# vovach777/llcomp

Measured on AMD Instinct MI355X. Metric: encode+decode MPix/s on 4K RGB8, bit-exact, higher is better.
Workload: dtype int32

## Files before the change

### llcomp_amd/csrc/model_kernels.hip

```cpp
#include <algorithm>

#include "device_common.hpp"
#include "kernels.hpp"

namespace llcomp_mi {

namespace {

constexpr int kMW = 256;
constexpr int kMH = 32;

template <int C>
__device__ __forceinline__ void rct_forward(const uint8_t* p, int16_t (&o)[C]) {
    if constexpr (C >= 3) {
        const int g = p[1], cb = int(p[2]) - g, cr = int(p[0]) - g;
        o[0] = int16_t(cr);
        o[1] = int16_t(g + (cb + cr) / 4);
        o[2] = int16_t(cb);
        if constexpr (C == 4) o[3] = p[3];
    } else {
#pragma unroll
        for (int k = 0; k < C; ++k) o[k] = p[k];
    }
}
// ... 651 lines not shown
struct RowTile {
    unsigned long long base;
    uint32_t sw;
};
template <int C>
__device__ __forceinline__ void load_row_tiles(const Geometry& g, uint32_t first_tile, uint32_t ntiles, RowTile* tiles) {
    if (threadIdx.x < ntiles) {
        const uint32_t tile = first_tile + threadIdx.x;
        const uint32_t per_frame = g.ntx * g.nty;
        const uint32_t frame = tile / per_frame, rem = tile - frame * per_frame;
        const uint32_t y = rem / g.ntx, tx = rem - y * g.ntx;
        const uint32_t x0 = tx * g.tile_w;
        tiles[threadIdx.x].base = ((size_t(frame) * g.h + y) * g.w + x0) * C;
        tiles[threadIdx.x].sw = g.w - x0 < g.tile_w ? g.w - x0 : g.tile_w;
    }
}

typedef short s16x2 __attribute__((ext_vector_type(2)));
typedef unsigned short u16x2 __attribute__((ext_vector_type(2)));
__device__ __forceinline__ u16x2 pk_min_u16(u16x2 a, u16x2 b) {
    u16x2 d;
    asm("v_pk_min_u16 %0, %1, %2" : "=v"(d) : "v"(a), "v"(b));
    return d;
}

template <int C>
__global__ __launch_bounds__(256) void k_model_rows_fwd(const Geometry g, const uint8_t* __restrict__ px,
                                                        uint16_t* __restrict__ lanes) {
    constexpr int K = 64, RUN = (K + 2) * C, TPG = 64 / C + 2;
    constexpr int RUNW = (RUN + 3) / 4 + 1;
    constexpr int PADL = (C - 1 + 1) & ~1, OCOLS = (PADL + 64 + C - 1 + 1) & ~1;
    __shared__ uint32_t raw[TPG][RUNW + 1];
    __shared__ __attribute__((aligned(4))) uint16_t otile[K][OCOLS];
    __shared__ RowTile tiles[TPG];
    const uint32_t chunks = (g.tile_w + K - 1) / K;
    uint32_t group, chunk;
    if (!xcd_group_chunk((g.n_slices + (1u << g.lane_shift) - 1) >> g.lane_shift, chunks, group, chunk)) return;
    const uint32_t k0 = chunk * K;
    const uint32_t gw = 1u << g.lane_shift;
    const uint32_t first_id = group << g.lane_shift;
    const uint32_t end_id = first_id + gw < g.n_slices ? first_id + gw : g.n_slices;
    const uint32_t first_tile = first_id / C, ntiles = (end_id - 1) / C - first_tile + 1;
    load_row_tiles<C>(g, first_tile, ntiles, tiles);
    __syncthreads();
    const size_t total_bytes = size_t(g.frames) * g.h * g.w * C;
    const uint32_t lane = threadIdx.x & 63, wave = threadIdx.x >> 6;
    constexpr int TPW = (TPG + 3) / 4, DPT = (RUNW + 63) / 64;
    uint32_t got[TPW][DPT];
#pragma unroll
    for (int t = 0; t < TPW; ++t) {
        const uint32_t tt = wave + 4 * t;
#pragma unroll
        for (int e = 0; e < DPT; ++e) got[t][e] = 0;
        if (tt < ntiles) {
            const long long start = (long long)tiles[tt].base + (long long)(int(k0) - 2) * C;
            const unsigned long long a0u = (unsigned long long)(start & ~3ll);
            const long long a0 = (long long)((unsigned long long)uint32_t(__builtin_amdgcn_readfirstlane(uint32_t(a0u))) |
                                             ((unsigned long long)uint32_t(__builtin_amdgcn_readfirstlane(uint32_t(a0u >> 32))) << 32));
            if (a0 >= 0 && size_t(a0) + 4 * size_t(RUNW) <= total_bytes) {
#pragma unroll
                for (int e = 0; e < DPT; ++e) {
                    const uint32_t d = lane + 64 * e;
                    if (d < uint32_t(RUNW)) __builtin_memcpy(&got[t][e], px + a0 + 4 * d, 4);
                }
            } else {
#pragma unroll
                for (int e = 0; e < DPT; ++e) {
                    const long long al = a0 + 4ll * (lane + 64 * e);
                    if (al >= 0 && size_t(al) + 4 <= total_bytes) __builtin_memcpy(&got[t][e], px + al, 4);
                    else if (al >= 0 && size_t(al) < total_bytes) got[t][e] = load_bytes_le(px + al, uint32_t(total_bytes - size_t(al)));
                }
            }
        }
    }
#pragma unroll
    for (int t = 0; t < TPW; ++t) {
        const uint32_t tt = wave + 4 * t;
#pragma unroll
        for (int e = 0; e < DPT; ++e) {
            const uint32_t d = lane + 64 * e;
            if (tt < ntiles && d < uint32_t(RUNW)) raw[tt][d] = got[t][e];
        }
    }
    __syncthreads();
    const uint32_t q = threadIdx.x & 7;
    const bool small = (g.flags & kGeoSmallModel) != 0;
    for (uint32_t tt = threadIdx.x >> 3; tt < ntiles; tt += 32) {
        const uint32_t sw = tiles[tt].sw;
        const uint32_t kb = k0 + 8 * q;
        if (kb >= sw) continue;
        const uint32_t skew = uint32_t(((long long)tiles[tt].base + (long long)(int(k0) - 2) * C) & 3);
        const uint8_t* p = reinterpret_cast<const uint8_t*>(&raw[tt][0]) + skew + 8 * q * C;
        s16x2 V[C][5];
#pragma unroll
        for (int j = 0; j < 5; ++j) {
            const uint8_t* a = p + 2 * j * C;
            if constexpr (C >= 3) {
                const s16x2 R = {short(a[0]), short(a[C])}, G = {short(a[1]), short(a[C + 1])}, B = {short(a[2]), short(a[C + 2])};
                const s16x2 cr = R - G, cb = B - G, sum = cb + cr;
                V[0][j] = cr;
                V[1][j] = G + ((sum + ((sum >> 15) & short(3))) >> 2);
                V[2][j] = cb;
                if constexpr (C == 4) V[3][j] = s16x2{short(a[3]), short(a[C + 3])};
            } else {
#pragma unroll
                for (int ch = 0; ch < C; ++ch) V[ch][j] = s16x2{short(a[ch]), short(a[C + ch])};
            }
        }
        uint32_t first_mask = ~0u;
        if (kb == 0) {
            first_mask = 0;
#pragma unroll
            for (int ch = 0; ch < C; ++ch) V[ch][0] = s16x2{128, 128};
        }
        if (small) first_mask = 0;
        const uint32_t colp = uint32_t(int((first_tile + tt) * C) - int(first_id) + PADL);
#pragma unroll
        for (int m = 0; m < 4; ++m) {
#pragma unroll
            for (int ch = 0; ch < C; ++ch) {
                const s16x2 cur = V[ch][m + 1], Lp = V[ch][m];
                const s16x2 lp = {V[ch][m].y, V[ch][m + 1].x};
                s16x2 dq = Lp - lp;
                uint32_t dqb = __builtin_bit_cast(uint32_t, dq) & ((m == 0 || small) ? first_mask : ~0u);
                dq = __builtin_bit_cast(s16x2, dqb);
                const s16x2 neg = dq >> 15;
                const u16x2 aq = __builtin_bit_cast(u16x2, (dq ^ neg) - neg);
                const u16x2 one = {1, 1};
                const u16x2 cidx = pk_min_u16(aq, one) + pk_min_u16(aq >> 2, one);
                const s16x2 res = ((cur - lp) ^ neg) - neg;
                const u16x2 sym = (__builtin_bit_cast(u16x2, res) & (unsigned short)0xFFF) + (cidx << 12);
                otile[8 * q + 2 * m][colp + ch] = sym.x;
                otile[8 * q + 2 * m + 1][colp + ch] = sym.y;
            }
        }
    }
    __syncthreads();
    if (g.lane_shift == 6) {
        for (uint32_t i = threadIdx.x; i < uint32_t(K) * 32; i += 256) {
            const uint32_t kk = i >> 5, d = i & 31, k = k0 + kk;
            if (k < g.tile_w)
                *reinterpret_cast<uint32_t*>(lanes + lane_order_index(g, first_id + 2 * d, k)) =
                    *reinterpret_cast<const uint32_t*>(&otile[kk][PADL + 2 * d]);
        }
    } else {
        for (uint32_t i = threadIdx.x; i < uint32_t(K) * gw; i += 256) {
            const uint32_t kk = i / gw, col = i - kk * gw, k = k0 + kk;
            if (k < g.tile_w && first_id + col < end_id) lanes[lane_order_index(g, first_id + col, k)] = otile[kk][PADL + col];
        }
    }
}

template <int C>
__global__ __launch_bounds__(256) void k_model_rows_inv(const Geometry g, const int16_t* __restrict__ lanes,
                                                        uint8_t* __restrict__ px) {
    constexpr int K = 64, TPG = 64 / C + 2;
    __shared__ __attribute__((aligned(4))) int16_t tile[K][64 + C + 1 + ((C + 1) & 1)];
    __shared__ RowTile tiles[TPG];
    const uint32_t chunks = (g.tile_w + K - 1) / K;
    uint32_t group, chunk;
    if (!xcd_chunk_group((g.n_slices + (1u << g.lane_shift) - 1) >> g.lane_shift, chunks, group, chunk)) return;
    const uint32_t k0 = chunk * K;
    const uint32_t gw = 1u << g.lane_shift;
    const uint32_t first_id = group << g.lane_shift;
    const uint32_t end_id = first_id + gw < g.n_slices ? first_id + gw : g.n_slices;
    const uint32_t first_tile = (first_id + C - 1) / C;
    const uint32_t end_tile = (end_id + C - 1) / C;
    if (first_tile >= end_tile) return;
    const uint32_t ntiles = end_tile - first_tile;
    load_row_tiles<C>(g, first_tile, ntiles, tiles);
    {
        uint32_t w[K * 32 / 256];
#pragma unroll
        for (int it = 0; it < K * 32 / 256; ++it) {
            const uint32_t i = threadIdx.x + 256 * it, kk = i >> 5, d = i & 31, k = k0 + kk;
            w[it] = 0;
            if (k < g.tile_w && g.lane_shift == 6)
                w[it] = *reinterpret_cast<const uint32_t*>(lanes + lane_order_index(g, first_id + 2 * d, k));
        }
        static_assert(K * (C - 1) <= 256, "one extra lane sample per thread");
        const uint32_t xk = threadIdx.x / (C > 1 ? C - 1 : 1), xe = threadIdx.x - xk * (C - 1);
        int16_t x = 0;
        if constexpr (C > 1) {
            const uint32_t id = first_id + gw + xe;
            if (xk < uint32_t(K) && id < g.n_slices && k0 + xk < g.tile_w) x = lanes[lane_order_index(g, id, k0 + xk)];
        }
#pragma unroll
        for (int it = 0; it < K * 32 / 256; ++it) {
            const uint32_t i = threadIdx.x + 256 * it, kk = i >> 5, d = i & 31;
            *reinterpret_cast<uint32_t*>(&tile[kk][2 * d]) = w[it];
        }
        if (g.lane_shift != 6) {
            __syncthreads();
            for (uint32_t i = threadIdx.x; i < uint32_t(K) * gw; i += 256) {
                const uint32_t kk = i / gw, col = i - kk * gw, k = k0 + kk;
                tile[kk][col] = (first_id + col < g.n_slices && k < g.tile_w) ? lanes[lane_order_index(g, first_id + col, k)] : int16_t(0);
            }
        }
        if constexpr (C > 1) {
            if (xk < uint32_t(K)) tile[xk][gw + xe] = x;
        }
    }
    __syncthreads();
    const uint32_t col0 = first_tile * C - first_id;
    const uint32_t q4 = threadIdx.x & 15;
    for (uint32_t tt = threadIdx.x >> 4; tt < ntiles; tt += 16) {
        const uint32_t sw = tiles[tt].sw, kb = k0 + 4 * q4;
        if (kb >= sw) continue;
        uint8_t bytes[4 * C];
#pragma unroll
        for (int i = 0; i < 4; ++i) {
            const int16_t* s = &tile[4 * q4 + i][col0 + tt * C];
            if constexpr (C >= 3) {
                int r = s[0], gg = s[1], bb = s[2];
                gg -= (r + bb) / 4;
                r += gg;
                bb += gg;
                bytes[i * C + 0] = uint8_t(min(max(r, 0), 255));
                bytes[i * C + 1] = uint8_t(min(max(gg, 0), 255));
                bytes[i * C + 2] = uint8_t(min(max(bb, 0), 255));
                if constexpr (C == 4) bytes[i * C + 3] = uint8_t(s[3]);
            } else {
#pragma unroll
                for (int c = 0; c < C; ++c) bytes[i * C + c] = uint8_t(s[c]);
            }
        }
        uint8_t* o = px + tiles[tt].base + size_t(kb) * C;
        const uint32_t npx = sw - kb < 4 ? sw - kb : 4;
        if (npx == 4) {
            uint32_t w[C];
#pragma unroll
            for (int c = 0; c < C; ++c)
                w[c] = uint32_t(bytes[4 * c]) | (uint32_t(bytes[4 * c + 1]) << 8) | (uint32_t(bytes[4 * c + 2]) << 16) |
                       (uint32_t(bytes[4 * c + 3]) << 24);
            __builtin_memcpy(o, w, 4 * C);
        } else {
            for (uint32_t i = 0; i < npx * C; ++i) o[i] = bytes[i];
        }
    }
}

struct RowTileCrop {
    long long base;
    uint32_t klo, khi;
};
template <int C>
__device__ __forceinline__ void load_row_tiles_crop(const Geometry& g, uint32_t first_tile, uint32_t ntiles, const Crop& cr,
                                                    RowTileCrop* tiles) {
    if (threadIdx.x < ntiles) {
        const uint32_t tile = first_tile + threadIdx.x;
        const uint32_t per_frame = g.ntx * g.nty;
        const uint32_t frame = tile / per_frame, rem = tile - frame * per_frame;
        const uint32_t y = rem / g.ntx, tx = rem - y * g.ntx;
        const uint32_t x0 = tx * g.tile_w;
        const uint32_t sw = g.w - x0 < g.tile_w ? g.w - x0 : g.tile_w;
        const uint32_t klo = cr.x0 > x0 ? cr.x0 - x0 : 0u;
        uint32_t khi = cr.x0 + cr.rw > x0 ? min(sw, cr.x0 + cr.rw - x0) : 0u;
        if (y < cr.y0 || y >= cr.y0 + cr.rh || khi <= klo) khi = 0;
        tiles[threadIdx.x].base = ((long long)(size_t(frame) * cr.rh + (y - cr.y0)) * cr.rw + (long long)x0 - (long long)cr.x0) * C;
        tiles[threadIdx.x].klo = klo;
        tiles[threadIdx.x].khi = khi;
    }
}
template <int C>
__global__ __launch_bounds__(256) void k_model_rows_inv_crop(const Geometry g, const int16_t* __restrict__ lanes,
                                                             uint8_t* __restrict__ px, const Crop cr) {
    constexpr int K = 64, TPG = 64 / C + 2;
    __shared__ __attribute__((aligned(4))) int16_t tile[K][64 + C + 1 + ((C + 1) & 1)];
    __shared__ RowTileCrop tiles[TPG];
    const uint32_t chunks = (g.tile_w + K - 1) / K;
    uint32_t group, chunk;
    if (!xcd_chunk_group((g.n_slices + (1u << g.lane_shift) - 1) >> g.lane_shift, chunks, group, chunk)) return;
    const uint32_t k0 = chunk * K;
    const uint32_t gw = 1u << g.lane_shift;
    const uint32_t first_id = group << g.lane_shift;
    const uint32_t end_id = first_id + gw < g.n_slices ? first_id + gw : g.n_slices;
    const uint32_t first_tile = (first_id + C - 1) / C;
    const uint32_t end_tile = (end_id + C - 1) / C;
    if (first_tile >= end_tile) return;
    const uint32_t ntiles = end_tile - first_tile;
    load_row_tiles_crop<C>(g, first_tile, ntiles, cr, tiles);
    {
        uint32_t w[K * 32 / 256];
#pragma unroll
        for (int it = 0; it < K * 32 / 256; ++it) {
            const uint32_t i = threadIdx.x + 256 * it, kk = i >> 5, d = i & 31, k = k0 + kk;
            w[it] = 0;
            if (k < g.tile_w && g.lane_shift == 6)
                w[it] = *reinterpret_cast<const uint32_t*>(lanes + lane_order_index(g, first_id + 2 * d, k));
        }
#pragma unroll
        for (int it = 0; it < K * 32 / 256; ++it) {
            const uint32_t i = threadIdx.x + 256 * it, kk = i >> 5, d = i & 31;
            *reinterpret_cast<uint32_t*>(&tile[kk][2 * d]) = w[it];
        }
    }
    if (g.lane_shift != 6) {
        __syncthreads();
        for (uint32_t i = threadIdx.x; i < uint32_t(K) * gw; i += 256) {
            const uint32_t kk = i / gw, col = i - kk * gw, k = k0 + kk;
            tile[kk][col] = (first_id + col < g.n_slices && k < g.tile_w) ? lanes[lane_order_index(g, first_id + col, k)] : int16_t(0);
        }
    }
    if constexpr (C > 1) {
        for (uint32_t i = threadIdx.x; i < uint32_t(K) * (C - 1); i += 256) {
            const uint32_t kk = i / (C - 1), e = i - kk * (C - 1), k = k0 + kk;
            const uint32_t id = first_id + gw + e;
            tile[kk][gw + e] = (id < g.n_slices && k < g.tile_w) ? lanes[lane_order_index(g, id, k)] : int16_t(0);
        }
    }
    __syncthreads();
    const uint32_t col0 = first_tile * C - first_id;
    const uint32_t q4 = threadIdx.x & 15;
    for (uint32_t tt = threadIdx.x >> 4; tt < ntiles; tt += 16) {
        const uint32_t sw = tiles[tt].khi, klo = tiles[tt].klo, kb = k0 + 4 * q4;
        if (kb >= sw || kb + 4 <= klo) continue;
        uint8_t bytes[4 * C];
#pragma unroll
        for (int i = 0; i < 4; ++i) {
            const int16_t* s = &tile[4 * q4 + i][col0 + tt * C];
            if constexpr (C >= 3) {
                int r = s[0], gg = s[1], bb = s[2];
                gg -= (r + bb) / 4;
                r += gg;
                bb += gg;
                bytes[i * C + 0] = uint8_t(min(max(r, 0), 255));
                bytes[i * C + 1] = uint8_t(min(max(gg, 0), 255));
                bytes[i * C + 2] = uint8_t(min(max(bb, 0), 255));
                if constexpr (C == 4) bytes[i * C + 3] = uint8_t(s[3]);
            } else {
#pragma unroll
                for (int c = 0; c < C; ++c) bytes[i * C + c] = uint8_t(s[c]);
            }
        }
        const uint32_t npx = sw - kb < 4 ? sw - kb : 4;
        if (npx < 4 || kb < klo) {
            for (uint32_t i = kb < klo ? klo - kb : 0u; i < npx; ++i)
                for (uint32_t c = 0; c < uint32_t(C); ++c) px[tiles[tt].base + (long long)(kb + i) * C + c] = bytes[i * C + c];
            continue;
        }
        uint32_t w[C];
#pragma unroll
        for (int c = 0; c < C; ++c)
            w[c] = uint32_t(bytes[4 * c]) | (uint32_t(bytes[4 * c + 1]) << 8) | (uint32_t(bytes[4 * c + 2]) << 16) |
                   (uint32_t(bytes[4 * c + 3]) << 24);
        __builtin_memcpy(px + tiles[tt].base + size_t(kb) * C, w, 4 * C);
    }
}



__global__ __launch_bounds__(256) void k_regions_index(const Geometry full, const Geometry sub, const RegionsFrame* __restrict__ tab,
                                                       const uint32_t* __restrict__ slice_len, const uint64_t* __restrict__ group_off,
                                                       uint32_t* __restrict__ sub_len, uint64_t* __restrict__ sub_off) {
    const uint32_t j = blockIdx.x * 256 + threadIdx.x;
    if (j >= sub.n_slices) return;
    const uint32_t id = regions_full_id(full, sub, tab, j);
    unsigned long long o = group_off[id >> full.lane_shift];
    for (uint32_t i = id & ~((1u << full.lane_shift) - 1); i < id; ++i) o += slice_len[i];
    sub_len[j] = slice_len[id];
    sub_off[j] = o;
}

template <int C>
__global__ __launch_bounds__(256) void k_model_inv_crops(const Geometry g, const int16_t* __restrict__ rec, uint8_t* __restrict__ px,
                                                         const RegionsFrame* __restrict__ tab, uint32_t rw, uint32_t rh, size_t npix) {
    const uint32_t c = C ? uint32_t(C) : g.c;
    const size_t per_frame = size_t(rw) * rh;
    for (size_t i = size_t(blockIdx.x) * blockDim.x + threadIdx.x; i < npix; i += size_t(gridDim.x) * blockDim.x) {
        const uint32_t f = uint32_t(i / per_frame);
        const uint32_t rem = uint32_t(i - f * per_frame), yy = rem / rw, xx = rem - yy * rw;
        const uint32_t y = tab[f].cy0 + yy, x = tab[f].cx0 + xx;
        uint8_t* o = px + (size_t(tab[f].out) * per_frame + rem) * c;
        uint32_t k = 0;
        if (c >= 3) {
            int r = rec[sample_index(g, f, y, x, 0)], gg = rec[sample_index(g, f, y, x, 1)], b = rec[sample_index(g, f, y, x, 2)];
            gg -= (r + b) / 4;
            r += gg;
            b += gg;
            o[0] = uint8_t(min(max(r, 0), 255));
            o[1] = uint8_t(min(max(gg, 0), 255));
            o[2] = uint8_t(min(max(b, 0), 255));
            k = 3;
        }
        for (; k < c; ++k) o[k] = uint8_t(rec[sample_index(g, f, y, x, k)]);
    }
}

template <int C>
__device__ __forceinline__ void load_row_tiles_crops(const Geometry& g, uint32_t first_tile, uint32_t ntiles, const RegionsFrame* tab,
                                                     uint32_t rw, uint32_t rh, RowTileCrop* tiles) {
    if (threadIdx.x < ntiles) {
        const uint32_t tile = first_tile + threadIdx.x;
        const uint32_t per_frame = g.ntx * g.nty;
        const uint32_t frame = tile / per_frame, rem = tile - frame * per_frame;
        const uint32_t y = rem / g.ntx, tx = rem - y * g.ntx;
        const uint32_t x0 = tx * g.tile_w;
        const uint32_t sw = g.w - x0 < g.tile_w ? g.w - x0 : g.tile_w;
        const uint32_t cx0 = tab[frame].cx0, cy0 = tab[frame].cy0;
        const uint32_t klo = cx0 > x0 ? cx0 - x0 : 0u;
        uint32_t khi = cx0 + rw > x0 ? min(sw, cx0 + rw - x0) : 0u;
        if (y < cy0 || y >= cy0 + rh || khi <= klo) khi = 0;
        tiles[threadIdx.x].base = ((long long)(size_t(tab[frame].out) * rh + (y - cy0)) * rw + (long long)x0 - (long long)cx0) * C;
        tiles[threadIdx.x].klo = klo;
        tiles[threadIdx.x].khi = khi;
    }
}
template <int C>
__global__ __launch_bounds__(256) void k_model_rows_inv_crops(const Geometry g, const int16_t* __restrict__ lanes,
                                                              uint8_t* __restrict__ px, const RegionsFrame* __restrict__ tab,
                                                              uint32_t rw, uint32_t rh) {
    constexpr int K = 64, TPG = 64 / C + 2;
    __shared__ __attribute__((aligned(4))) int16_t tile[K][64 + C + 1 + ((C + 1) & 1)];
    __shared__ RowTileCrop tiles[TPG];
    const uint32_t chunks = (g.tile_w + K - 1) / K;
    uint32_t group, chunk;
    if (!xcd_chunk_group((g.n_slices + (1u << g.lane_shift) - 1) >> g.lane_shift, chunks, group, chunk)) return;
    const uint32_t k0 = chunk * K;
    const uint32_t gw = 1u << g.lane_shift;
    const uint32_t first_id = group << g.lane_shift;
    const uint32_t end_id = first_id + gw < g.n_slices ? first_id + gw : g.n_slices;
    const uint32_t first_tile = (first_id + C - 1) / C;
    const uint32_t end_tile = (end_id + C - 1) / C;
    if (first_tile >= end_tile) return;
    const uint32_t ntiles = end_tile - first_tile;
    load_row_tiles_crops<C>(g, first_tile, ntiles, tab, rw, rh, tiles);
    {
        uint32_t w[K * 32 / 256];
#pragma unroll
        for (int it = 0; it < K * 32 / 256; ++it) {
            const uint32_t i = threadIdx.x + 256 * it, kk = i >> 5, d = i & 31, k = k0 + kk;
            w[it] = 0;
            if (k < g.tile_w && g.lane_shift == 6)
                w[it] = *reinterpret_cast<const uint32_t*>(lanes + lane_order_index(g, first_id + 2 * d, k));
        }
#pragma unroll
        for (int it = 0; it < K * 32 / 256; ++it) {
            const uint32_t i = threadIdx.x + 256 * it, kk = i >> 5, d = i & 31;
            *reinterpret_cast<uint32_t*>(&tile[kk][2 * d]) = w[it];
        }
    }
    if (g.lane_shift != 6) {
        __syncthreads();
        for (uint32_t i = threadIdx.x; i < uint32_t(K) * gw; i += 256) {
            const uint32_t kk = i / gw, col = i - kk * gw, k = k0 + kk;
            tile[kk][col] = (first_id + col < g.n_slices && k < g.tile_w) ? lanes[lane_order_index(g, first_id + col, k)] : int16_t(0);
        }
    }
    if constexpr (C > 1) {
        for (uint32_t i = threadIdx.x; i < uint32_t(K) * (C - 1); i += 256) {
            const uint32_t kk = i / (C - 1), e = i - kk * (C - 1), k = k0 + kk;
            const uint32_t id = first_id + gw + e;
            tile[kk][gw + e] = (id < g.n_slices && k < g.tile_w) ? lanes[lane_order_index(g, id, k)] : int16_t(0);
        }
    }
    __syncthreads();
    const uint32_t col0 = first_tile * C - first_id;
    const uint32_t q4 = threadIdx.x & 15;
    for (uint32_t tt = threadIdx.x >> 4; tt < ntiles; tt += 16) {
        const uint32_t sw = tiles[tt].khi, klo = tiles[tt].klo, kb = k0 + 4 * q4;
        if (kb >= sw || kb + 4 <= klo) continue;
        uint8_t bytes[4 * C];
#pragma unroll
        for (int i = 0; i < 4; ++i) {
            const int16_t* s = &tile[4 * q4 + i][col0 + tt * C];
            if constexpr (C >= 3) {
                int r = s[0], gg = s[1], bb = s[2];
                gg -= (r + bb) / 4;
                r += gg;
                bb += gg;
                bytes[i * C + 0] = uint8_t(min(max(r, 0), 255));
                bytes[i * C + 1] = uint8_t(min(max(gg, 0), 255));
                bytes[i * C + 2] = uint8_t(min(max(bb, 0), 255));
                if constexpr (C == 4) bytes[i * C + 3] = uint8_t(s[3]);
            } else {
#pragma unroll
                for (int c = 0; c < C; ++c) bytes[i * C + c] = uint8_t(s[c]);
            }
        }
        const uint32_t npx = sw - kb < 4 ? sw - kb : 4;
        if (npx < 4 || kb < klo) {
            for (uint32_t i = kb < klo ? klo - kb : 0u; i < npx; ++i)
                for (uint32_t c = 0; c < uint32_t(C); ++c) px[tiles[tt].base + (long long)(kb + i) * C + c] = bytes[i * C + c];
            continue;
        }
        uint32_t w[C];
#pragma unroll
        for (int c = 0; c < C; ++c)
            w[c] = uint32_t(bytes[4 * c]) | (uint32_t(bytes[4 * c + 1]) << 8) | (uint32_t(bytes[4 * c + 2]) << 16) |
                   (uint32_t(bytes[4 * c + 3]) << 24);
        __builtin_memcpy(px + tiles[tt].base + size_t(kb) * C, w, 4 * C);
    }
}


}

#define LLMI_DISPATCH_C(c, CALL) \
    switch (c) {                 \
        case 1: { constexpr int C = 1; CALL; } break; \
        case 2: { constexpr int C = 2; CALL; } break; \
        case 3: { constexpr int C = 3; CALL; } break; \
        case 4: { constexpr int C = 4; CALL; } break; \
        default: return hipErrorInvalidValue; \
    }

hipError_t launch_model_fwd(const Geometry& g, const uint8_t* d_px, uint32_t* d_sym, hipStream_t stream) {
    if (g.c > 4) {
        const size_t npix = size_t(g.frames) * g.h * g.w;
        k_model_fwd_any<<<dim3(uint32_t((npix + 255) / 256)), dim3(256), 0, stream>>>(g, d_px, d_sym, npix);
        return hipGetLastError();
    }
    const uint32_t nbx = (g.w + kMW - 1) / kMW;
    const uint32_t spt = (g.tile_h + kMH - 1) / kMH;
    const uint64_t blocks = uint64_t(nbx) * spt * g.nty * g.frames;
    if (blocks == 0 || blocks > 0x7FFFFFFFull) return hipErrorInvalidValue;
    LLMI_DISPATCH_C(g.c, (k_model_fwd<C><<<dim3(uint32_t(blocks)), dim3(kMW), 0, stream>>>(g, d_px, d_sym)));
    return hipGetLastError();
}

uint32_t lane_groups(const Geometry& g) { return (g.n_slices + (1u << g.lane_shift) - 1) >> g.lane_shift; }
uint32_t slice_capacity_samples(const Geometry& g) { return g.slice_samples; }

hipError_t launch_to_lane_order_u32(const Geometry& g, const uint32_t* d_img, uint32_t* d_lanes, hipStream_t stream) {
    const uint32_t max_n = slice_capacity_samples(g);
    const uint64_t blocks = uint64_t(lane_groups(g)) * ((max_n + 63) / 64);
    if (blocks == 0 || blocks > 0x7FFFFFFFull) return hipErrorInvalidValue;
    k_to_lane_order<uint32_t><<<dim3(uint32_t(blocks)), dim3(256), 0, stream>>>(g, max_n, d_img, d_lanes);
    return hipGetLastError();
}

hipError_t launch_from_lane_order_i16(const Geometry& g, const int16_t* d_lanes, int16_t* d_img, hipStream_t stream) {
    const uint32_t max_n = slice_capacity_samples(g);
    const uint64_t blocks = uint64_t(lane_groups(g)) * ((max_n + 63) / 64);
    if (blocks == 0 || blocks > 0x7FFFFFFFull) return hipErrorInvalidValue;
    k_from_lane_order<int16_t><<<dim3(uint32_t(blocks)), dim3(256), 0, stream>>>(g, max_n, d_lanes, d_img);
    return hipGetLastError();
}

bool model_is_fused(const Geometry& g) { return g.planar && rows_mode(g) && g.c <= 4; }
bool rows_encoder_reads_pixels(const Geometry& g) {
    return model_is_fused(g) && (uint64_t(63 / g.c + 2) * g.tile_w * g.c + 4 < (1ull << 31));
}

hipError_t launch_model_rows_fwd(const Geometry& g, const uint8_t* d_px, uint16_t* d_lanes, hipStream_t stream) {
    const uint64_t blocks = xcd_grid(lane_groups(g), (g.tile_w + 63) / 64);
    if (blocks == 0 || blocks > 0x7FFFFFFFull) return hipErrorInvalidValue;
    LLMI_DISPATCH_C(g.c, (k_model_rows_fwd<C><<<dim3(uint32_t(blocks)), dim3(256), 0, stream>>>(g, d_px, d_lanes)));
    return hipGetLastError();
}

hipError_t launch_model_rows_inv(const Geometry& g, const int16_t* d_lanes, uint8_t* d_px, hipStream_t stream) {
    const uint64_t blocks = xcd_chunk_grid(lane_groups(g), (g.tile_w + 63) / 64);
    if (blocks == 0 || blocks > 0x7FFFFFFFull) return hipErrorInvalidValue;
    LLMI_DISPATCH_C(g.c, (k_model_rows_inv<C><<<dim3(uint32_t(blocks)), dim3(256), 0, stream>>>(g, d_lanes, d_px)));
    return hipGetLastError();
}

hipError_t launch_model_inv(const Geometry& g, const int16_t* d_rec, uint8_t* d_px, hipStream_t stream) {
    const size_t npix = size_t(g.frames) * g.h * g.w;
    if (g.c > 4) {
        k_model_inv_any<<<dim3(uint32_t((npix + 255) / 256)), dim3(256), 0, stream>>>(g, d_rec, d_px, npix);
        return hipGetLastError();
    }
    const uint32_t blocks = uint32_t(std::min<size_t>((npix + 255) / 256, 256 * 16));
    LLMI_DISPATCH_C(g.c, (k_model_inv<C><<<dim3(blocks), dim3(256), 0, stream>>>(g, d_rec, d_px, npix)));
    return hipGetLastError();
}

hipError_t launch_group_sums(const Geometry& g, const uint32_t* d_slice_len, uint64_t* d_group_off, hipStream_t stream) {
    k_group_sums<<<dim3((g.n_slices + kSumThreads - 1) / kSumThreads), dim3(kSumThreads), 0, stream>>>(d_slice_len, g.n_slices, g.lane_shift, d_group_off);
    return hipGetLastError();
}

hipError_t launch_frame_bytes(const Geometry& g, const uint32_t* d_slice_len, uint64_t* d_frame_bytes, hipStream_t stream) {
    k_frame_bytes<<<dim3(g.frames), dim3(256), 0, stream>>>(d_slice_len, g.slices_per_frame, d_frame_bytes);
    return hipGetLastError();
}

hipError_t launch_scan_groups(const Geometry& g, uint64_t* d_group_off, uint64_t* d_total, hipStream_t stream) {
    k_scan_groups<<<dim3(1), dim3(kScanThreads), 0, stream>>>(d_group_off, lane_groups(g), d_total);
    return hipGetLastError();
}

hipError_t launch_copy_segments(const uint8_t* d_src, uint8_t* d_dst, const uint64_t* d_src_off, const uint64_t* d_dst_off,
                                const uint64_t* d_len, uint32_t n_seg, uint64_t max_len, hipStream_t stream) {
    if (n_seg == 0) return hipSuccess;
    if (n_seg > 65535) return hipErrorInvalidValue;
    const uint64_t pieces = (max_len / 4 + kSegPieceDwords - 1) / kSegPieceDwords;
    const uint32_t gx = uint32_t(std::min<uint64_t>(std::max<uint64_t>(pieces, 1), 1024));
    k_copy_segments<<<dim3(gx, n_seg), dim3(256), 0, stream>>>(d_src, d_dst, d_src_off, d_dst_off, d_len);
    return hipGetLastError();
}

hipError_t launch_range_sums(const uint32_t* d_vals, const uint64_t* d_start, const uint64_t* d_count, uint64_t* d_out, uint32_t n,
                             uint32_t cap, hipStream_t stream) {
    if (!n) return hipSuccess;
    k_range_sums<<<dim3(n), dim3(256), 0, stream>>>(d_vals, d_start, d_count, d_out, cap);
    return hipGetLastError();
}

hipError_t launch_pack_payload(const Geometry& g, const uint8_t* d_units, const uint32_t* d_slice_len,
                               const uint64_t* d_offsets, uint8_t* d_payload, uint64_t payload_cap,
                               uint32_t* d_status, hipStream_t stream) {
    k_pack_payload<<<dim3(lane_groups(g)), dim3(256), 0, stream>>>(g, reinterpret_cast<const uint4*>(d_units), d_slice_len,
                                                                   d_offsets, d_payload, payload_cap, d_status);
    return hipGetLastError();
}

hipError_t launch_region_index(const Geometry& full, const Geometry& sub, const RegionBox& box, const uint32_t* d_slice_len,
                               const uint64_t* d_group_off, uint32_t* d_sub_len, uint64_t* d_sub_off, hipStream_t stream) {
    if (sub.n_slices == 0) return hipErrorInvalidValue;
    k_region_index<<<dim3((sub.n_slices + 255) / 256), dim3(256), 0, stream>>>(full, sub, box, d_slice_len, d_group_off, d_sub_len, d_sub_off);
    return hipGetLastError();
}

hipError_t launch_stage_region_streams(const Geometry& sub, const uint8_t* d_payload, uint64_t payload_bytes, const uint32_t* d_sub_len,
                                       const uint64_t* d_sub_off, uint8_t* d_units, uint32_t* d_status, hipStream_t stream) {
    k_stage_region_streams<<<dim3(lane_groups(sub)), dim3(256), 0, stream>>>(sub, d_payload, payload_bytes, d_sub_len, d_sub_off,
                                                                             reinterpret_cast<uint4*>(d_units), d_status);
    return hipGetLastError();
}

hipError_t launch_model_inv_crop(const Geometry& sub, const int16_t* d_rec, uint8_t* d_px, const Crop& cr, hipStream_t stream) {
    const size_t npix = size_t(sub.frames) * cr.rh * cr.rw;
    if (npix == 0 || uint64_t(cr.x0) + cr.rw > sub.w || uint64_t(cr.y0) + cr.rh > sub.h) return hipErrorInvalidValue;
    const uint32_t blocks = uint32_t(std::min<size_t>((npix + 255) / 256, 256 * 16));
    switch (sub.c) {
        case 1: k_model_inv_crop<1><<<dim3(blocks), dim3(256), 0, stream>>>(sub, d_rec, d_px, cr, npix); break;
        case 2: k_model_inv_crop<2><<<dim3(blocks), dim3(256), 0, stream>>>(sub, d_rec, d_px, cr, npix); break;
        case 3: k_model_inv_crop<3><<<dim3(blocks), dim3(256), 0, stream>>>(sub, d_rec, d_px, cr, npix); break;
        case 4: k_model_inv_crop<4><<<dim3(blocks), dim3(256), 0, stream>>>(sub, d_rec, d_px, cr, npix); break;
        default: k_model_inv_crop<0><<<dim3(blocks), dim3(256), 0, stream>>>(sub, d_rec, d_px, cr, npix); break;
    }
    return hipGetLastError();
}

hipError_t launch_model_rows_inv_crop(const Geometry& sub, const int16_t* d_lanes, uint8_t* d_px, const Crop& cr, hipStream_t stream) {
    if (!cr.rw || !cr.rh || uint64_t(cr.x0) + cr.rw > sub.w || uint64_t(cr.y0) + cr.rh > sub.h) return hipErrorInvalidValue;
    const uint64_t blocks = xcd_chunk_grid(lane_groups(sub), (sub.tile_w + 63) / 64);
    if (blocks == 0 || blocks > 0x7FFFFFFFull) return hipErrorInvalidValue;
    LLMI_DISPATCH_C(sub.c, (k_model_rows_inv_crop<C><<<dim3(uint32_t(blocks)), dim3(256), 0, stream>>>(sub, d_lanes, d_px, cr)));
    return hipGetLastError();
}

// ... 41 lines not shown
```

Measured before the change: 29580.

## Transpose rows-inverse LDS tile to lane-major swizzled layout with packed-int16 RCT

```diff
diff --git a/llcomp_amd/csrc/model_kernels.hip b/llcomp_amd/csrc/model_kernels.hip
--- a/llcomp_amd/csrc/model_kernels.hip
+++ b/llcomp_amd/csrc/model_kernels.hip
@@ -827,91 +827,154 @@
 }
 
 template <int C>
+struct RowsInv {
+    static constexpr int K = 64;
+    static constexpr int LANES = 64 + C - 1;
+    static constexpr int TPG = 64 / C + 2;
+};
+__device__ __forceinline__ uint32_t rows_inv_at(uint32_t L, uint32_t s) {
+    return (L << 6) + (((s >> 2) ^ (L & 14u)) << 2) + (s & 3u);
+}
+struct RowsInvBlock {
+    uint32_t group, k0, first_id, first_tile, ntiles, col0;
+};
+template <int C>
+__device__ __forceinline__ bool rows_inv_block(const Geometry& g, RowsInvBlock& b) {
+    const uint32_t chunks = (g.tile_w + RowsInv<C>::K - 1) / RowsInv<C>::K;
+    uint32_t chunk;
+    if (!xcd_chunk_group((g.n_slices + (1u << g.lane_shift) - 1) >> g.lane_shift, chunks, b.group, chunk)) return false;
+    b.k0 = chunk * RowsInv<C>::K;
+    const uint32_t gw = 1u << g.lane_shift;
+    b.first_id = b.group << g.lane_shift;
+    const uint32_t end_id = b.first_id + gw < g.n_slices ? b.first_id + gw : g.n_slices;
+    b.first_tile = (b.first_id + C - 1) / C;
+    const uint32_t end_tile = (end_id + C - 1) / C;
+    if (b.first_tile >= end_tile) return false;
+    b.ntiles = end_tile - b.first_tile;
+    b.col0 = b.first_tile * C - b.first_id;
+    return true;
+}
+template <int C>
+__device__ __forceinline__ void rows_inv_fill(const Geometry& g, const int16_t* __restrict__ lanes, const RowsInvBlock& b, int16_t* tile) {
+    constexpr int K = RowsInv<C>::K;
+    const uint32_t gw = 1u << g.lane_shift, k0 = b.k0;
+    static_assert(K * (C - 1) <= 256, "one extra lane sample per thread");
+    const uint32_t xk = threadIdx.x / (C > 1 ? C - 1 : 1), xe = threadIdx.x - xk * (C - 1);
+    if (g.lane_shift == 6) {
+        const uint32_t d = threadIdx.x & 31, s0 = (threadIdx.x >> 5) * 8;
+        const int16_t* piece = lanes + ((size_t(b.group) * g.slice_samples + k0) << 6) + (s0 * 64 + 2 * d);
+        uint32_t w[8];
+        if (k0 + K <= g.tile_w) {
+#pragma unroll
+            for (int it = 0; it < 8; ++it) w[it] = *reinterpret_cast<const uint32_t*>(piece + 64 * it);
+        } else {
+#pragma unroll
+            for (int it = 0; it < 8; ++it) {
+                w[it] = 0;
+                if (k0 + s0 + it < g.tile_w) w[it] = *reinterpret_cast<const uint32_t*>(piece + 64 * it);
+            }
+        }
+        int16_t x = 0;
+        if constexpr (C > 1) {
+            const uint32_t id = b.first_id + gw + xe;
+            if (xk < uint32_t(K) && id < g.n_slices && k0 + xk < g.tile_w) x = lanes[lane_order_index(g, id, k0 + xk)];
+        }
+        uint4 even, odd;
+        even.x = __builtin_amdgcn_perm(w[1], w[0], 0x05040100u), odd.x = __builtin_amdgcn_perm(w[1], w[0], 0x07060302u);
+        even.y = __builtin_amdgcn_perm(w[3], w[2], 0x05040100u), odd.y = __builtin_amdgcn_perm(w[3], w[2], 0x07060302u);
+        even.z = __builtin_amdgcn_perm(w[5], w[4], 0x05040100u), odd.z = __builtin_amdgcn_perm(w[5], w[4], 0x07060302u);
+        even.w = __builtin_amdgcn_perm(w[7], w[6], 0x05040100u), odd.w = __builtin_amdgcn_perm(w[7], w[6], 0x07060302u);
+        *reinterpret_cast<uint4*>(tile + rows_inv_at(2 * d, s0)) = even;
+        *reinterpret_cast<uint4*>(tile + rows_inv_at(2 * d + 1, s0)) = odd;
+        if constexpr (C > 1) {
+            if (xk < uint32_t(K)) tile[rows_inv_at(gw + xe, xk)] = x;
+        }
+    } else {
+        for (uint32_t i = threadIdx.x; i < uint32_t(K) * gw; i += 256) {
+            const uint32_t kk = i / gw, col = i - kk * gw, k = k0 + kk;
+            tile[rows_inv_at(col, kk)] =
+                (b.first_id + col < g.n_slices && k < g.tile_w) ? lanes[lane_order_index(g, b.first_id + col, k)] : int16_t(0);
+        }
+        if constexpr (C > 1) {
+            const uint32_t id = b.first_id + gw + xe;
+            if (xk < uint32_t(K))
+                tile[rows_inv_at(gw + xe, xk)] = (id < g.n_slices && k0 + xk < g.tile_w) ? lanes[lane_order_index(g, id, k0 + xk)] : int16_t(0);
+        }
+    }
+}
+
+__device__ __forceinline__ uint32_t sat_pk_u8_i16(s16x2 a) {
+    uint32_t d;
+    asm("v_sat_pk_u8_i16 %0, %1" : "=v"(d) : "v"(a));
+    return d;
+}
+template <int C>
+__device__ __forceinline__ void rows_inv_pixels(const int16_t* tile, uint32_t L0, uint32_t q4, uint32_t (&w)[C]) {
+    s16x2 P[C][2];
+#pragma unroll
+    for (int c = 0; c < C; ++c) {
+        const uint2 v = *reinterpret_cast<const uint2*>(tile + rows_inv_at(L0 + c, 4 * q4));
+        P[c][0] = __builtin_bit_cast(s16x2, v.x);
+        P[c][1] = __builtin_bit_cast(s16x2, v.y);
+    }
+    if constexpr (C >= 3) {
+        uint32_t R[2], G[2], B[2];
+#pragma unroll
+        for (int j = 0; j < 2; ++j) {
+            const s16x2 r = P[0][j], gg = P[1][j], bb = P[2][j];
+            const s16x2 x = r ^ bb, h = (r & bb) + (x >> 1);
+            const s16x2 neg = __builtin_bit_cast(s16x2, __builtin_bit_cast(u16x2, h) >> 15);
+            const s16x2 t = (h >> 1) + ((h | x) & neg);
+            R[j] = sat_pk_u8_i16(__builtin_elementwise_add_sat(r - t, gg));
+            G[j] = sat_pk_u8_i16(__builtin_elementwise_sub_sat(gg, t));
+            B[j] = sat_pk_u8_i16(__builtin_elementwise_add_sat(bb - t, gg));
+        }
+        if constexpr (C == 3) {
+            w[0] = __builtin_amdgcn_perm(B[0], __builtin_amdgcn_perm(G[0], R[0], 0x010c0400u), 0x03040100u);
+            w[1] = __builtin_amdgcn_perm(B[0], G[0], 0x0c0c0501u) | __builtin_amdgcn_perm(G[1], R[1], 0x04000c0cu);
+            w[2] = __builtin_amdgcn_perm(B[1], __builtin_amdgcn_perm(G[1], R[1], 0x0c05010cu), 0x05020104u);
+        } else {
+#pragma unroll
+            for (int j = 0; j < 2; ++j) {
+                const uint32_t rg = __builtin_amdgcn_perm(G[j], R[j], 0x05010400u);
+                const uint32_t ba = __builtin_amdgcn_perm(__builtin_bit_cast(uint32_t, P[3][j]), B[j], 0x06010400u);
+                w[2 * j] = __builtin_amdgcn_perm(ba, rg, 0x05040100u);
+                w[2 * j + 1] = __builtin_amdgcn_perm(ba, rg, 0x07060302u);
+            }
+        }
+    } else if constexpr (C == 2) {
+        w[0] = __builtin_amdgcn_perm(__builtin_bit_cast(uint32_t, P[1][0]), __builtin_bit_cast(uint32_t, P[0][0]), 0x06020400u);
+        w[1] = __builtin_amdgcn_perm(__builtin_bit_cast(uint32_t, P[1][1]), __builtin_bit_cast(uint32_t, P[0][1]), 0x06020400u);
+    } else {
+        w[0] = __builtin_amdgcn_perm(__builtin_bit_cast(uint32_t, P[0][1]), __builtin_bit_cast(uint32_t, P[0][0]), 0x06040200u);
+    }
+}
+template <int C>
+__device__ __forceinline__ void rows_inv_store_some(uint8_t* o, const uint32_t (&w)[C], uint32_t p0, uint32_t p1) {
+#pragma unroll
+    for (int j = 0; j < 4 * C; ++j)
+        if (uint32_t(j) >= p0 * C && uint32_t(j) < p1 * C) o[j] = uint8_t(w[j >> 2] >> (8 * (j & 3)));
+}
+
+template <int C>
 __global__ __launch_bounds__(256) void k_model_rows_inv(const Geometry g, const int16_t* __restrict__ lanes,
                                                         uint8_t* __restrict__ px) {
-    constexpr int K = 64, TPG = 64 / C + 2;
-    __shared__ __attribute__((aligned(4))) int16_t tile[K][64 + C + 1 + ((C + 1) & 1)];
-    __shared__ RowTile tiles[TPG];
-    const uint32_t chunks = (g.tile_w + K - 1) / K;
-    uint32_t group, chunk;
-    if (!xcd_chunk_group((g.n_slices + (1u << g.lane_shift) - 1) >> g.lane_shift, chunks, group, chunk)) return;
-    const uint32_t k0 = chunk * K;
-    const uint32_t gw = 1u << g.lane_shift;
-    const uint32_t first_id = group << g.lane_shift;
-    const uint32_t end_id = first_id + gw < g.n_slices ? first_id + gw : g.n_slices;
-    const uint32_t first_tile = (first_id + C - 1) / C;
-    const uint32_t end_tile = (end_id + C - 1) / C;
-    if (first_tile >= end_tile) return;
-    const uint32_t ntiles = end_tile - first_tile;
-    load_row_tiles<C>(g, first_tile, ntiles, tiles);
-    {
-        uint32_t w[K * 32 / 256];
-#pragma unroll
-        for (int it = 0; it < K * 32 / 256; ++it) {
-            const uint32_t i = threadIdx.x + 256 * it, kk = i >> 5, d = i & 31, k = k0 + kk;
-            w[it] = 0;
-            if (k < g.tile_w && g.lane_shift == 6)
-                w[it] = *reinterpret_cast<const uint32_t*>(lanes + lane_order_index(g, first_id + 2 * d, k));
-        }
-        static_assert(K * (C - 1) <= 256, "one extra lane sample per thread");
-        const uint32_t xk = threadIdx.x / (C > 1 ? C - 1 : 1), xe = threadIdx.x - xk * (C - 1);
-        int16_t x = 0;
-        if constexpr (C > 1) {
-            const uint32_t id = first_id + gw + xe;
-            if (xk < uint32_t(K) && id < g.n_slices && k0 + xk < g.tile_w) x = lanes[lane_order_index(g, id, k0 + xk)];
-        }
-#pragma unroll
-        for (int it = 0; it < K * 32 / 256; ++it) {
-            const uint32_t i = threadIdx.x + 256 * it, kk = i >> 5, d = i & 31;
-            *reinterpret_cast<uint32_t*>(&tile[kk][2 * d]) = w[it];
-        }
-        if (g.lane_shift != 6) {
-            __syncthreads();
-            for (uint32_t i = threadIdx.x; i < uint32_t(K) * gw; i += 256) {
-                const uint32_t kk = i / gw, col = i - kk * gw, k = k0 + kk;
-                tile[kk][col] = (first_id + col < g.n_slices && k < g.tile_w) ? lanes[lane_order_index(g, first_id + col, k)] : int16_t(0);
-            }
-        }
-        if constexpr (C > 1) {
-            if (xk < uint32_t(K)) tile[xk][gw + xe] = x;
-        }
-    }
-    __syncthreads();
-    const uint32_t col0 = first_tile * C - first_id;
+    __shared__ __attribute__((aligned(16))) int16_t tile[RowsInv<C>::LANES * RowsInv<C>::K];
+    __shared__ RowTile tiles[RowsInv<C>::TPG];
+    RowsInvBlock b;
+    if (!rows_inv_block<C>(g, b)) return;
+    load_row_tiles<C>(g, b.first_tile, b.ntiles, tiles);
+    rows_inv_fill<C>(g, lanes, b, tile);
+    __syncthreads();
     const uint32_t q4 = threadIdx.x & 15;
-    for (uint32_t tt = threadIdx.x >> 4; tt < ntiles; tt += 16) {
-        const uint32_t sw = tiles[tt].sw, kb = k0 + 4 * q4;
+    for (uint32_t tt = threadIdx.x >> 4; tt < b.ntiles; tt += 16) {
+        const uint32_t sw = tiles[tt].sw, kb = b.k0 + 4 * q4;
         if (kb >= sw) continue;
-        uint8_t bytes[4 * C];
-#pragma unroll
-        for (int i = 0; i < 4; ++i) {
-            const int16_t* s = &tile[4 * q4 + i][col0 + tt * C];
-            if constexpr (C >= 3) {
-                int r = s[0], gg = s[1], bb = s[2];
-                gg -= (r + bb) / 4;
-                r += gg;
-                bb += gg;
-                bytes[i * C + 0] = uint8_t(min(max(r, 0), 255));
-                bytes[i * C + 1] = uint8_t(min(max(gg, 0), 255));
-                bytes[i * C + 2] = uint8_t(min(max(bb, 0), 255));
-                if constexpr (C == 4) bytes[i * C + 3] = uint8_t(s[3]);
-            } else {
-#pragma unroll
-                for (int c = 0; c < C; ++c) bytes[i * C + c] = uint8_t(s[c]);
-            }
-        }
+        uint32_t w[C];
+        rows_inv_pixels<C>(tile, b.col0 + tt * C, q4, w);
         uint8_t* o = px + tiles[tt].base + size_t(kb) * C;
-        const uint32_t npx = sw - kb < 4 ? sw - kb : 4;
-        if (npx == 4) {
-            uint32_t w[C];
-#pragma unroll
-            for (int c = 0; c < C; ++c)
-                w[c] = uint32_t(bytes[4 * c]) | (uint32_t(bytes[4 * c + 1]) << 8) | (uint32_t(bytes[4 * c + 2]) << 16) |
-                       (uint32_t(bytes[4 * c + 3]) << 24);
-            __builtin_memcpy(o, w, 4 * C);
-        } else {
-            for (uint32_t i = 0; i < npx * C; ++i) o[i] = bytes[i];
-        }
+        if (sw - kb >= 4) __builtin_memcpy(o, w, 4 * C);
+        else rows_inv_store_some<C>(o, w, 0, sw - kb);
     }
 }
 
@@ -938,89 +1001,29 @@
     }
 }
 template <int C>
+__device__ __forceinline__ void rows_inv_store_crop(const RowsInvBlock& b, const int16_t* tile, const RowTileCrop* tiles, uint8_t* __restrict__ px) {
+    const uint32_t q4 = threadIdx.x & 15;
+    for (uint32_t tt = threadIdx.x >> 4; tt < b.ntiles; tt += 16) {
+        const uint32_t khi = tiles[tt].khi, klo = tiles[tt].klo, kb = b.k0 + 4 * q4;
+        if (kb >= khi || kb + 4 <= klo) continue;
+        uint32_t w[C];
+        rows_inv_pixels<C>(tile, b.col0 + tt * C, q4, w);
+        uint8_t* o = px + (tiles[tt].base + (long long)kb * C);
+        if (khi - kb >= 4 && kb >= klo) __builtin_memcpy(o, w, 4 * C);
+        else rows_inv_store_some<C>(o, w, kb < klo ? klo - kb : 0u, khi - kb < 4 ? khi - kb : 4u);
+    }
+}
+template <int C>
 __global__ __launch_bounds__(256) void k_model_rows_inv_crop(const Geometry g, const int16_t* __restrict__ lanes,
                                                              uint8_t* __restrict__ px, const Crop cr) {
-    constexpr int K = 64, TPG = 64 / C + 2;
-    __shared__ __attribute__((aligned(4))) int16_t tile[K][64 + C + 1 + ((C + 1) & 1)];
-    __shared__ RowTileCrop tiles[TPG];
-    const uint32_t chunks = (g.tile_w + K - 1) / K;
-    uint32_t group, chunk;
-    if (!xcd_chunk_group((g.n_slices + (1u << g.lane_shift) - 1) >> g.lane_shift, chunks, group, chunk)) return;
-    const uint32_t k0 = chunk * K;
-    const uint32_t gw = 1u << g.lane_shift;
-    const uint32_t first_id = group << g.lane_shift;
-    const uint32_t end_id = first_id + gw < g.n_slices ? first_id + gw : g.n_slices;
-    const uint32_t first_tile = (first_id + C - 1) / C;
-    const uint32_t end_tile = (end_id + C - 1) / C;
-    if (first_tile >= end_tile) return;
-    const uint32_t ntiles = end_tile - first_tile;
-    load_row_tiles_crop<C>(g, first_tile, ntiles, cr, tiles);
-    {
-        uint32_t w[K * 32 / 256];
-#pragma unroll
-        for (int it = 0; it < K * 32 / 256; ++it) {
-            const uint32_t i = threadIdx.x + 256 * it, kk = i >> 5, d = i & 31, k = k0 + kk;
-            w[it] = 0;
-            if (k < g.tile_w && g.lane_shift == 6)
-                w[it] = *reinterpret_cast<const uint32_t*>(lanes + lane_order_index(g, first_id + 2 * d, k));
-        }
-#pragma unroll
-        for (int it = 0; it < K * 32 / 256; ++it) {
-            const uint32_t i = threadIdx.x + 256 * it, kk = i >> 5, d = i & 31;
-            *reinterpret_cast<uint32_t*>(&tile[kk][2 * d]) = w[it];
-        }
-    }
-    if (g.lane_shift != 6) {
-        __syncthreads();
-        for (uint32_t i = threadIdx.x; i < uint32_t(K) * gw; i += 256) {
-            const uint32_t kk = i / gw, col = i - kk * gw, k = k0 + kk;
-            tile[kk][col] = (first_id + col < g.n_slices && k < g.tile_w) ? lanes[lane_order_index(g, first_id + col, k)] : int16_t(0);
-        }
-    }
-    if constexpr (C > 1) {
-        for (uint32_t i = threadIdx.x; i < uint32_t(K) * (C - 1); i += 256) {
-            const uint32_t kk = i / (C - 1), e = i - kk * (C - 1), k = k0 + kk;
-            const uint32_t id = first_id + gw + e;
-            tile[kk][gw + e] = (id < g.n_slices && k < g.tile_w) ? lanes[lane_order_index(g, id, k)] : int16_t(0);
-        }
-    }
-    __syncthreads();
-    const uint32_t col0 = first_tile * C - first_id;
-    const uint32_t q4 = threadIdx.x & 15;
-    for (uint32_t tt = threadIdx.x >> 4; tt < ntiles; tt += 16) {
-        const uint32_t sw = tiles[tt].khi, klo = tiles[tt].klo, kb = k0 + 4 * q4;
-        if (kb >= sw || kb + 4 <= klo) continue;
-        uint8_t bytes[4 * C];
-#pragma unroll
-        for (int i = 0; i < 4; ++i) {
-            const int16_t* s = &tile[4 * q4 + i][col0 + tt * C];
-            if constexpr (C >= 3) {
-                int r = s[0], gg = s[1], bb = s[2];
-                gg -= (r + bb) / 4;
-                r += gg;
-                bb += gg;
-                bytes[i * C + 0] = uint8_t(min(max(r, 0), 255));
-                bytes[i * C + 1] = uint8_t(min(max(gg, 0), 255));
-                bytes[i * C + 2] = uint8_t(min(max(bb, 0), 255));
-                if constexpr (C == 4) bytes[i * C + 3] = uint8_t(s[3]);
-            } else {
-#pragma unroll
-                for (int c = 0; c < C; ++c) bytes[i * C + c] = uint8_t(s[c]);
-            }
-        }
-        const uint32_t npx = sw - kb < 4 ? sw - kb : 4;
-        if (npx < 4 || kb < klo) {
-            for (uint32_t i = kb < klo ? klo - kb : 0u; i < npx; ++i)
-                for (uint32_t c = 0; c < uint32_t(C); ++c) px[tiles[tt].base + (long long)(kb + i) * C + c] = bytes[i * C + c];
-            continue;
-        }
-        uint32_t w[C];
-#pragma unroll
-        for (int c = 0; c < C; ++c)
-            w[c] = uint32_t(bytes[4 * c]) | (uint32_t(bytes[4 * c + 1]) << 8) | (uint32_t(bytes[4 * c + 2]) << 16) |
-                   (uint32_t(bytes[4 * c + 3]) << 24);
-        __builtin_memcpy(px + tiles[tt].base + size_t(kb) * C, w, 4 * C);
-    }
+    __shared__ __attribute__((aligned(16))) int16_t tile[RowsInv<C>::LANES * RowsInv<C>::K];
+    __shared__ RowTileCrop tiles[RowsInv<C>::TPG];
+    RowsInvBlock b;
+    if (!rows_inv_block<C>(g, b)) return;
+    load_row_tiles_crop<C>(g, b.first_tile, b.ntiles, cr, tiles);
+    rows_inv_fill<C>(g, lanes, b, tile);
+    __syncthreads();
+    rows_inv_store_crop<C>(b, tile, tiles, px);
 }
 
 
@@ -1085,87 +1088,14 @@
 __global__ __launch_bounds__(256) void k_model_rows_inv_crops(const Geometry g, const int16_t* __restrict__ lanes,
                                                               uint8_t* __restrict__ px, const RegionsFrame* __restrict__ tab,
                                                               uint32_t rw, uint32_t rh) {
-    constexpr int K = 64, TPG = 64 / C + 2;
-    __shared__ __attribute__((aligned(4))) int16_t tile[K][64 + C + 1 + ((C + 1) & 1)];
-    __shared__ RowTileCrop tiles[TPG];
-    const uint32_t chunks = (g.tile_w + K - 1) / K;
-    uint32_t group, chunk;
-    if (!xcd_chunk_group((g.n_slices + (1u << g.lane_shift) - 1) >> g.lane_shift, chunks, group, chunk)) return;
-    const uint32_t k0 = chunk * K;
-    const uint32_t gw = 1u << g.lane_shift;
-    const uint32_t first_id = group << g.lane_shift;
-    const uint32_t end_id = first_id + gw < g.n_slices ? first_id + gw : g.n_slices;
-    const uint32_t first_tile = (first_id + C - 1) / C;
-    const uint32_t end_tile = (end_id + C - 1) / C;
-    if (first_tile >= end_tile) return;
-    const uint32_t ntiles = end_tile - first_tile;
-    load_row_tiles_crops<C>(g, first_tile, ntiles, tab, rw, rh, tiles);
-    {
-        uint32_t w[K * 32 / 256];
-#pragma unroll
-        for (int it = 0; it < K * 32 / 256; ++it) {
-            const uint32_t i = threadIdx.x + 256 * it, kk = i >> 5, d = i & 31, k = k0 + kk;
-            w[it] = 0;
-            if (k < g.tile_w && g.lane_shift == 6)
-                w[it] = *reinterpret_cast<const uint32_t*>(lanes + lane_order_index(g, first_id + 2 * d, k));
-        }
-#pragma unroll
-        for (int it = 0; it < K * 32 / 256; ++it) {
-            const uint32_t i = threadIdx.x + 256 * it, kk = i >> 5, d = i & 31;
-            *reinterpret_cast<uint32_t*>(&tile[kk][2 * d]) = w[it];
-        }
-    }
-    if (g.lane_shift != 6) {
-        __syncthreads();
-        for (uint32_t i = threadIdx.x; i < uint32_t(K) * gw; i += 256) {
-            const uint32_t kk = i / gw, col = i - kk * gw, k = k0 + kk;
-            tile[kk][col] = (first_id + col < g.n_slices && k < g.tile_w) ? lanes[lane_order_index(g, first_id + col, k)] : int16_t(0);
-        }
-    }
-    if constexpr (C > 1) {
-        for (uint32_t i = threadIdx.x; i < uint32_t(K) * (C - 1); i += 256) {
-            const uint32_t kk = i / (C - 1), e = i - kk * (C - 1), k = k0 + kk;
-            const uint32_t id = first_id + gw + e;
-            tile[kk][gw + e] = (id < g.n_slices && k < g.tile_w) ? lanes[lane_order_index(g, id, k)] : int16_t(0);
-        }
-    }
-    __syncthreads();
-    const uint32_t col0 = first_tile * C - first_id;
-    const uint32_t q4 = threadIdx.x & 15;
-    for (uint32_t tt = threadIdx.x >> 4; tt < ntiles; tt += 16) {
-        const uint32_t sw = tiles[tt].khi, klo = tiles[tt].klo, kb = k0 + 4 * q4;
-        if (kb >= sw || kb + 4 <= klo) continue;
-        uint8_t bytes[4 * C];
-#pragma unroll
-        for (int i = 0; i < 4; ++i) {
-            const int16_t* s = &tile[4 * q4 + i][col0 + tt * C];
-            if constexpr (C >= 3) {
-                int r = s[0], gg = s[1], bb = s[2];
-                gg -= (r + bb) / 4;
-                r += gg;
-                bb += gg;
-                bytes[i * C + 0] = uint8_t(min(max(r, 0), 255));
-                bytes[i * C + 1] = uint8_t(min(max(gg, 0), 255));
-                bytes[i * C + 2] = uint8_t(min(max(bb, 0), 255));
-                if constexpr (C == 4) bytes[i * C + 3] = uint8_t(s[3]);
-            } else {
-#pragma unroll
-                for (int c = 0; c < C; ++c) bytes[i * C + c] = uint8_t(s[c]);
-            }
-        }
-        const uint32_t npx = sw - kb < 4 ? sw - kb : 4;
-        if (npx < 4 || kb < klo) {
-            for (uint32_t i = kb < klo ? klo - kb : 0u; i < npx; ++i)
-                for (uint32_t c = 0; c < uint32_t(C); ++c) px[tiles[tt].base + (long long)(kb + i) * C + c] = bytes[i * C + c];
-            continue;
-        }
-        uint32_t w[C];
-#pragma unroll
-        for (int c = 0; c < C; ++c)
-            w[c] = uint32_t(bytes[4 * c]) | (uint32_t(bytes[4 * c + 1]) << 8) | (uint32_t(bytes[4 * c + 2]) << 16) |
-                   (uint32_t(bytes[4 * c + 3]) << 24);
-        __builtin_memcpy(px + tiles[tt].base + size_t(kb) * C, w, 4 * C);
-    }
+    __shared__ __attribute__((aligned(16))) int16_t tile[RowsInv<C>::LANES * RowsInv<C>::K];
+    __shared__ RowTileCrop tiles[RowsInv<C>::TPG];
+    RowsInvBlock b;
+    if (!rows_inv_block<C>(g, b)) return;
+    load_row_tiles_crops<C>(g, b.first_tile, b.ntiles, tab, rw, rh, tiles);
+    rows_inv_fill<C>(g, lanes, b, tile);
+    __syncthreads();
+    rows_inv_store_crop<C>(b, tile, tiles, px);
 }
 
 
```

Result: slower. 28770 (-2.7%).
